# google/nerfactor

Hardware: AMD Instinct MI355X
Metric: rays/sec (NeRF coarse+fine render, 64+128 samples/ray) (higher is better)
Workload: dtype bf16; 1 GPU; lego_3072-shaped NeRF coarse+fine MLP render, 800x800 rays/view, 64+128 samples (BASELINE.json configs[1]); rays_per_view=640000, n_samples_coarse=64, n_samples_fine=128, kernel_variant=7

## Files before the change

nerfactor_amd/_capi.py:

```python
import ctypes
import os

import torch

_HERE = os.path.dirname(os.path.abspath(__file__))
LIB_PATH = os.path.join(_HERE, 'libnfx.so')
if os.environ.get('NFX_LIB_PATH'):
    LIB_PATH = os.environ['NFX_LIB_PATH']

PREC_BF16, PREC_FP32, PREC_FP32_NATIVE = 0, 1, 2
ACT_NONE, ACT_RELU, ACT_SIGMOID, ACT_SOFTPLUS = 0, 1, 2, 3
IN_XYZ, IN_XYZ_LDIR, IN_Z_RUSINK = 0, 1, 2

if not os.path.exists(LIB_PATH):
    raise ImportError(
        "%s not found: build it with `python -m nerfactor_amd.build` (or __graft_entry__.build()); "
        "nerfactor_amd has no fallback path." % LIB_PATH)

lib = ctypes.CDLL(LIB_PATH)

_p = ctypes.c_void_p
_i = ctypes.c_int
_i64 = ctypes.c_int64
_f = ctypes.c_float
# ... 45 lines not shown
    'nfx_nerf_mlp_bwd': (_i, [_p, _p, _p, _i64, _i, _p, _i, _p, _p, _sz, _pp, _pp, _p]),
    'nfx_brdf_train_packed_bytes': (_sz, []),
    'nfx_brdf_pack_train_weights': (_i, [_pp, _pp, _i, _i, _p, _sz]),
    'nfx_brdf_spec_bwd_workspace_bytes': (_sz, [_i, _i64]),
    'nfx_brdf_spec_bwd': (_i, [_p, _p, _p, _p, _i, _p, _i, _p, _i, _i64, _p, _p, _p, _p, _sz, _p]),
    'nfx_brdf_spec_bwd_list_bytes': (_sz, [_i64, _i]),
    'nfx_brdf_spec_bwd_rows': (_i, [_p, _p, _p, _p, _i, _p, _i, _p, _i, _i64, _p, _p, _p, _p, _sz, _p, _sz, _p]),
    'nfx_brdf_rows_fwd': (_i, [_p, _i, _p, _i64, _i, _p, _i, _p, _p]),
    'nfx_brdf_rows_bwd_workspace_bytes': (_sz, [_i, _i64, _i]),
    'nfx_brdf_rows_bwd': (_i, [_p, _i, _p, _i64, _i, _p, _i, _p, _p, _sz, _p, _pp, _pp, _p]),
    'nfx_shade_bwd_workspace_bytes': (_sz, [_i]),
    'nfx_shade_bwd': (_i, [_p, _p, _p, _p, _p, _p, _f, _f, _p, _p, _p, _p, _i64, _i, _i, _p, _p, _p, _p, _p, _p,
                           _p, _p, _sz, _p]),
    'nfx_l2_normalize_rows': (_i, [_p, _p, _i64, _i, _f, _p]),
    'nfx_l2_normalize_rows_bwd': (_i, [_p, _p, _p, _i64, _i, _f, _p]),
    'nfx_light_smoothness': (_i, [_p, _i, _i, _f, _f, _p, _p, _p]),
    'nfx_pair_loss_fwd': (_i, [_p, _i, _p, _f, _i64, _p, _p]),
    'nfx_pair_loss_bwd': (_i, [_p, _i, _p, _f, _i64, _p, _p]),
    'nfx_pack_gather': (_i, [_p, _p, _i64, _p, _p]),
    'nfx_amsgrad_step': (_i, [_p, _p, _p, _p, _p, _i64, _f, _f, _f, _f, _i64, _p]),
    'nfx_amsgrad_step_size': (_f, [_f, _f, _f, _i64]),
    'nfx_amsgrad_step_dev': (_i, [_p, _p, _p, _p, _p, _i64, _p, _f, _f, _f, _p]),
    'nfx_nerf_sigma_fwd': (_i, [_p, _p, _p, _i64, _i, _p, _i, _p, _p]),
    'nfx_lvis_fwd_rows': (_i, [_p, _p, _i64, _f, _p, _i, _p, _i, _p, _sz, _p, _p, _p, _p]),
    'nfx_zero_rows': (_i, [_p, _p, _i64, _i, _p]),
    'nfx_shade_fwd_rows': (_i, [_p, _p, _p, _p, _p, _p, _f, _f, _p, _p, _p, _p, _p, _i64, _i, _i, _i, _p, _p]),
    'nfx_shade_olat_fwd_rows': (_i, [_p, _p, _p, _p, _p, _p, _f, _f, _p, _p, _p, _p, _f, _f, _i64, _i, _i, _p, _p, _p, _p]),
    'nfx_nerf_refine_select': (_i, [_p, _p, _p, _i64, _i, _f, _f, _f, _f, _i, _p, _p, _p]),
    'nfx_nerf_sigma_refine': (_i, [_p, _p, _p, _i64, _i, _p, _p, _p, _p, _p]),
    'nfx_nerf_sigma_refine_last': (_i, [_p, _p, _p, _i64, _i, _p, _p, _p]),
    'nfx_nerf_sigma_fwd_list': (_i, [_p, _p, _p, _i64, _i, _p, _i, _p, _p, _p, _p]),
    'nfx_occgrid_workspace_bytes': (_sz, [_i64, _i]),
    'nfx_occgrid_select': (_i, [_p, _p, _p, _i64, _i, _p, _i, _p, _p, _p, _p, _sz, _p]),
    'nfx_occgrid_bake': (_i, [_p, _i, _i, _f, _i, _p, _p, _p]),
    'nfx_nerf_geom_packed_bytes': (_sz, [_i]),
    'nfx_nerf_pack_geom_weights': (_i, [_pp, _pp, _i, _p, _sz]),
    'nfx_nerf_sigma_grad': (_i, [_p, _p, _p, _i64, _i, _p, _i, _p, _p]),
    'nfx_nerf_sigma_grad_workspace_bytes': (_sz, [_i64, _i]),
    'nfx_nerf_sigma_grad_rows': (_i, [_p, _p, _p, _i64, _i, _p, _i, _p, _p, _sz, _p]),
    'nfx_selftest_mfma_bf16': (_i, [_p, _p, _p, _p]),
    'nfx_selftest_sincos': (_i, [_p, _i64, _i, _p, _p]),
    'nfx_selftest_tr16': (_i, [_p, _p, _p, _i, _p]),
    'nfx_selftest_wgrad_plan': (_i, [_i, _p, _p, _i64, _p, _p, _p, _p]),
    'nfx_selftest_wgrad_partial_bytes': (_sz, [_i, _p, _p, _i64]),
    'nfx_selftest_wgrad_batch': (_i, [_i, _pp, _pp, _p, _p, _pp, _pp, _i64, _i64, _p, _p, _sz, _p]),
    'nfx_mlp_generic_packed_bytes': (_sz, [_i, _i, _p, _p, _i]),
    'nfx_mlp_generic_pack': (_i, [_pp, _pp, _i, _i, _p, _p, _i, _p, _sz]),
    'nfx_mlp_generic_fwd': (_i, [_p, _i64, _i, _i, _i, _p, _p, _p, _p, _i, _p, _i, _i, _p]),
    'nfx_mlp_generic_train_packed_bytes': (_sz, [_i, _i, _p, _p, _i]),
    'nfx_mlp_generic_pack_train': (_i, [_pp, _pp, _i, _i, _p, _p, _i, _p, _sz]),
    'nfx_mlp_generic_bwd_workspace_bytes': (_sz, [_i64, _i, _i, _p, _p, _i]),
    'nfx_mlp_generic_split_hilo': (_i, [_p, _i, _i, _p, _p, _i, _p]),
    'nfx_brdf_rows_geom_fwd': (_i, [_p, _p, _p, _p, _i, _p, _i, _i64, _i, _p, _i, _p, _p]),
    'nfx_brdf_rows_geom_bwd': (_i, [_p, _p, _p, _i, _p, _i, _i64, _i, _p, _i, _p, _p, _p]),
    'nfx_embed_bwd': (_i, [_p, _i64, _i, _i, _p, _i, _i, _p, _p]),
    'nfx_mlp_generic_bwd': (_i, [_p, _i64, _i, _i, _i, _p, _p, _p, _p, _i, _p, _i, _i, _p, _i, _pp, _pp, _p, _sz, _p]),
    'nfx_embed': (_i, [_p, _p, _p, _i64, _i, _i, _i, _i, _p, _i, _i, _p]),
}

for _name, (_res, _args) in SIGNATURES.items():
    _fn = getattr(lib, _name)
    _fn.restype = _res
    _fn.argtypes = _args


class NfxError(RuntimeError):
    """Raised for any non-zero return of the C-ABI; mirrors how the reference surfaces failures as
    Python exceptions (tf.errors.InvalidArgumentError from tf.debugging.*)."""


def last_error():
    buf = ctypes.create_string_buffer(512)
    lib.nfx_last_error(buf, 512)
    return buf.value.decode()


def check(rc, what):
    if rc != 0:
        raise NfxError("%s failed (%d): %s" % (what, rc, last_error()))


OPTION_KEYS = ('nerf_variant', 'nerf_fold', 'nerf_blocks', 'm128_blocks', 'lvis_variant', 'brdf_variant', 'brdf_ct', 'nerf_bwd',
               'nerf_bwd_nw', 'm128_bwd', 'wgrad_lds', 'wgrad_slabs', 'wgrad_rounds', 'wgrad_narrow', 'wgrad_fused', 'lvis_verify', 'lvis_rows', 'brdf_bwd_rows', 'nerf_bwd_rows', 'sigma_grad_rows', 'sigma_variant',
               'sigma_x3_variant')


def set_option(key, value):
    check(lib.nfx_set_option(key.encode(), int(value)), 'nfx_set_option(%s)' % key)


def unset_option(key):
    check(lib.nfx_unset_option(key.encode()), 'nfx_unset_option(%s)' % key)


def get_option(key):
    v, isset = _i(0), _i(0)
    check(lib.nfx_get_option(key.encode(), ctypes.byref(v), ctypes.byref(isset)), 'nfx_get_option(%s)' % key)
    return v.value if isset.value else None


class option:

    def __init__(self, key, value):
        self.key, self.value = key, value

    def __enter__(self):
        self.prev = get_option(self.key)
        if self.value is None:
            unset_option(self.key)
        else:
            set_option(self.key, self.value)
        return self

    def __exit__(self, *exc):
        if self.prev is None:
            unset_option(self.key)
        else:
            set_option(self.key, self.prev)
        return False


for _k in OPTION_KEYS:
    _v = os.environ.get('NFX_' + _k.upper())
    if _v not in (None, ''):
        set_option(_k, int(_v))
```

nerfactor_amd/csrc/capi.cpp:

```cpp
#include <hip/hip_runtime.h>
#include <stdarg.h>
#include <stdio.h>
#include <stdlib.h>
#include <string.h>

#include <atomic>
#include <vector>

#include "capi_common.hpp"
#include "nerf_layout.hpp"
#include "nerf_fold_layout.hpp"
#include "pack.hpp"

static thread_local char g_err[512] = "";

int nfx_fail(int code, const char* fmt, ...) {
    va_list ap;
    va_start(ap, fmt);
    vsnprintf(g_err, sizeof(g_err), fmt, ap);
    va_end(ap);
    return code;
}
int nfx_hip_result(int e, const char* what) {
    if (e == 0) return NFX_OK;
    return nfx_fail(NFX_EHIP, "%s: HIP error %d (%s)", what, e, hipGetErrorString((hipError_t)e));
}

extern "C" {
int nfx_version(void) { return 100; }

int nfx_last_error(char* buf, size_t len) {
    if (!buf || len == 0) return NFX_EINVAL;
    strncpy(buf, g_err, len - 1);
    buf[len - 1] = 0;
    return NFX_OK;
}

namespace {
struct Option {
    const char* key;
    std::atomic<int> value;
    std::atomic<int> is_set;
};
Option g_options[] = {
    {"nerf_variant", {0}, {0}},
    {"nerf_fold", {0}, {0}},
    {"nerf_blocks", {0}, {0}},
    {"m128_blocks", {0}, {0}},
    {"lvis_variant", {0}, {0}},
    {"lvis_verify", {0}, {0}},
    {"lvis_rows", {0}, {0}},
    {"brdf_bwd_rows", {0}, {0}},
    {"sigma_variant", {0}, {0}},
    {"sigma_x3_variant", {0}, {0}},
    {"sigma_grad_rows", {0}, {0}},
    {"nerf_bwd_rows", {0}, {0}},
    {"brdf_variant", {0}, {0}},
    {"brdf_ct", {0}, {0}},
    {"nerf_bwd", {0}, {0}},
    {"nerf_bwd_nw", {0}, {0}},
    {"m128_bwd", {0}, {0}},
    {"wgrad_lds", {0}, {0}},
    {"wgrad_slabs", {0}, {0}},
    {"wgrad_rounds", {0}, {0}},
    {"wgrad_narrow", {0}, {0}},
    {"wgrad_fused", {0}, {0}},
    {"wgrad_splits", {0}, {0}},
    {"wgrad_map", {0}, {0}},
};
Option* find_option(const char* key) {
    if (!key) return nullptr;
    for (Option& o : g_options)
        if (strcmp(o.key, key) == 0) return &o;
    return nullptr;
}
}

int nfx_option_int(const char* key, int dflt) {
    Option* o = find_option(key);
    return o && o->is_set.load(std::memory_order_acquire) ? o->value.load(std::memory_order_relaxed) : dflt;
}
int nfx_set_option(const char* key, int value) {
    Option* o = find_option(key);
    if (!o) return nfx_fail(NFX_EINVAL, "nfx_set_option: unknown option '%s'", key ? key : "(null)");
    o->value.store(value, std::memory_order_relaxed);
    o->is_set.store(1, std::memory_order_release);
    return NFX_OK;
}
int nfx_unset_option(const char* key) {
    Option* o = find_option(key);
    if (!o) return nfx_fail(NFX_EINVAL, "nfx_unset_option: unknown option '%s'", key ? key : "(null)");
    o->is_set.store(0, std::memory_order_release);
    return NFX_OK;
}
int nfx_get_option(const char* key, int* value, int* is_set) {
    Option* o = find_option(key);
    if (!o || !value) return nfx_fail(NFX_EINVAL, "nfx_get_option: unknown option '%s' or null output", key ? key : "(null)");
    *value = o->value.load(std::memory_order_relaxed);
    if (is_set) *is_set = o->is_set.load(std::memory_order_acquire);
    return NFX_OK;
}

size_t nfx_nerf_packed_bytes(int prec) {
    if (prec == NFX_PREC_BF16) return nfx::nerf::kBlobBytes;
    if (prec == NFX_PREC_FP32) return (size_t)nfx::nerf::kBlobBytes + nfx::nerf::kWeightBytes;
    return 0;
}

static int pack_nerf_fragments(const float* const kernels[12], const float* const biases[12], uint8_t* w0, float* b) {
    using namespace nfx;
    using namespace nfx::pack;
    uint8_t* w = w0;
    const Seg pe_xyz{kPosEnc, 10, 0, nullptr};
    const Seg hid256{kHidden, 256, 0, nullptr};
    w += pack_layer_bf16({pe_xyz}, {{kernels[0], biases[0], 256}}, 8, 8, w, b + nerf::kBiasL0);
    for (int l = 1; l <= 7; ++l) {
        float* bl = b + nerf::kBiasL0 + 256 * l;
        if (l == 5) {
            const Seg pe_skip{kPosEnc, 10, 256, nullptr};
            w += pack_layer_bf16({hid256, pe_skip}, {{kernels[5], biases[5], 256}}, 8, 24, w, bl);
        } else {
            w += pack_layer_bf16({hid256}, {{kernels[l], biases[l], 256}}, 8, 16, w, bl);
        }
    }
    w += pack_layer_bf16({hid256}, {{kernels[9], biases[9], 256}, {kernels[8], biases[8], 1}}, 9, 16, w,
                         b + nerf::kBiasBott);
    const Seg pe_view{kPosEnc, 4, 256, nullptr};
    w += pack_layer_bf16({hid256, pe_view}, {{kernels[10], biases[10], 128}}, 4, 24, w, b + nerf::kBiasRgb0);
    const Seg hid128{kHidden, 128, 0, nullptr};
    w += pack_layer_bf16({hid128}, {{kernels[11], biases[11], 3}}, 1, 8, w, b + nerf::kBiasRgb1);
    return w == w0 + nerf::kWeightBytes ? NFX_OK : NFX_EINVAL;
}

int nfx_nerf_pack_weights(const float* const kernels[12], const float* const biases[12], int prec,
                          void* blob, size_t blob_bytes) {
    using namespace nfx;
    REQUIRE(kernels && biases && blob, "nfx_nerf_pack_weights: null argument");
// ... 78 lines not shown
        if (variant == 6)
            return nfx_hip_result(nfx_launch_nerf_mlp_bf16_v6(rayo, rayd, z, n_pts, n_samples, blob, rgbs, blocks,
                                                              0, (hipStream_t)stream),
                                  "nerf_mlp_fwd(bf16, v6)");
        if (variant != 0 && variant != 1)
            return nfx_fail(NFX_EINVAL, "nfx_nerf_mlp_fwd: NFX_NERF_VARIANT %d is not built (0, 1, 6, 7, 8)", variant);
        return nfx_hip_result(nfx_launch_nerf_mlp_bf16(rayo, rayd, z, n_pts, n_samples, blob, rgbs, variant,
                                                       blocks, (hipStream_t)stream),
                              "nerf_mlp_fwd(bf16)");
    }
    if (prec == NFX_PREC_FP32)
        return nfx_hip_result(nfx_launch_nerf_mlp_x3(rayo, rayd, z, n_pts, n_samples, blob, rgbs, blocks, (hipStream_t)stream),
                              "nerf_mlp_fwd(fp32 via 3 x bf16)");
    return nfx_fail(NFX_EINVAL, "nfx_nerf_mlp_fwd: bad prec %d", prec);
}

size_t nfx_nerf_fold_workspace_bytes(void) { return nfx::nerf::fold::kBlobBytes; }

int nfx_nerf_fold_blob(const void* blob, void* workspace, size_t workspace_bytes, void* stream) {
    REQUIRE(blob && workspace, "nfx_nerf_fold_blob: null pointer");
    REQUIRE(workspace_bytes >= nfx_nerf_fold_workspace_bytes(), "nfx_nerf_fold_blob: workspace too small (%zu < %zu)",
            workspace_bytes, nfx_nerf_fold_workspace_bytes());
    if (!ALIGNED(blob, 16) || !ALIGNED(workspace, 16))
        return nfx_fail(NFX_EALIGN, "nfx_nerf_fold_blob: blob and workspace must be 16-byte aligned");
    const uintptr_t b = (uintptr_t)blob, w = (uintptr_t)workspace;
    REQUIRE(b + nfx::nerf::kBlobBytes <= w || w + nfx_nerf_fold_workspace_bytes() <= b,
            "nfx_nerf_fold_blob: the workspace overlaps the blob");
    return nfx_hip_result(nfx_launch_nerf_fold(blob, workspace, (hipStream_t)stream), "nerf_fold_blob");
}

int nfx_nerf_mlp_fwd_folded(const float* rayo, const float* rayd, const float* z, int64_t n_rays, int n_samples,
                            const void* blob, void* workspace, size_t workspace_bytes, float* rgbs, void* stream) {
    REQUIRE(n_rays >= 0 && n_samples >= 1, "nfx_nerf_mlp_fwd_folded: bad shape (%lld rays, %d samples)",
            (long long)n_rays, n_samples);
    if (n_rays == 0) return NFX_OK;
    REQUIRE(rayo && rayd && z && blob && rgbs, "nfx_nerf_mlp_fwd_folded: null pointer");
    if (!ALIGNED(rgbs, 16)) return nfx_fail(NFX_EALIGN, "nfx_nerf_mlp_fwd_folded: rgbs must be 16-byte aligned");
    const int rc = nfx_nerf_fold_blob(blob, workspace, workspace_bytes, stream);
    if (rc) return rc;
    const long long n_pts = (long long)n_rays * n_samples;
    const int blocks = nfx_option_int("nerf_blocks", 256);
    const int variant = nfx_option_int("nerf_variant", 7);
    if (variant == 6 || variant == 7 || variant == 8)
        return nfx_hip_result(nfx_launch_nerf_mlp_bf16_v6_fold(rayo, rayd, z, n_pts, n_samples, workspace, rgbs, blocks,
                                                               variant == 8 ? 2 : variant == 7 ? 1 : 0, (hipStream_t)stream),
                              "nerf_mlp_fwd_folded(bf16, v6-8)");
    if (variant != 0 && variant != 1)
        return nfx_fail(NFX_EINVAL, "nfx_nerf_mlp_fwd_folded: NFX_NERF_VARIANT %d is not built (0, 1, 6, 7, 8)", variant);
    return nfx_hip_result(nfx_launch_nerf_mlp_bf16_fold(rayo, rayd, z, n_pts, n_samples, workspace, rgbs, variant, blocks,
                                                        (hipStream_t)stream),
                          "nerf_mlp_fwd_folded(bf16)");
}

int nfx_composite_fwd(const float* rgbs, const float* z, const float* rayd, const float* noise,
                      int64_t n_rays, int n_samples, int white_bg, float* rgb, float* occu, float* depth,
                      float* disp, float* weights, void* stream) {
    REQUIRE(n_rays >= 0 && n_samples >= 1, "nfx_composite_fwd: bad shape");
    if (n_rays == 0) return NFX_OK;
    REQUIRE(rgbs && z && rayd, "nfx_composite_fwd: null input");
    if (!ALIGNED(rgbs, 16)) return nfx_fail(NFX_EALIGN, "nfx_composite_fwd: rgbs must be 16-byte aligned");
    return nfx_hip_result(nfx_launch_composite(rgbs, z, rayd, noise, n_rays, n_samples, white_bg, rgb, occu,
                                               depth, disp, weights, (hipStream_t)stream),
                          "composite_fwd");
}

int nfx_nerf_surface_fwd(const float* sigma, const float* z, const float* rayo, const float* rayd, int64_t n_rays,
                         int n_samples, float occu_thres, int quantize_alpha, float* alpha, float* xyz, float* depth,
                         float* occu, void* stream) {
    REQUIRE(n_rays >= 0 && n_samples >= 1, "nfx_nerf_surface_fwd: bad shape (%lld rays, %d samples)", (long long)n_rays,
            n_samples);
    REQUIRE(occu_thres == occu_thres, "nfx_nerf_surface_fwd: occu_thres is NaN");
    if (n_rays == 0) return NFX_OK;
    REQUIRE(sigma && z && rayo && rayd, "nfx_nerf_surface_fwd: null input");
    REQUIRE(alpha && xyz && depth, "nfx_nerf_surface_fwd: null output (only occu may be NULL)");
    return nfx_hip_result(nfx_launch_surface(sigma, z, rayo, rayd, n_rays, n_samples, occu_thres, quantize_alpha ? 1 : 0, alpha,
                                             xyz, depth, occu, (hipStream_t)stream),
                          "nerf_surface_fwd");
}

int nfx_sample_fine(const float* z, const float* weights, int64_t n_rays, int n_coarse, int n_fine,
                    const float* u, float* z_all, void* stream) {
    REQUIRE(n_rays >= 0, "nfx_sample_fine: n_rays < 0");
    REQUIRE(n_coarse <= 258, "nfx_sample_fine: at most 258 coarse samples (256 pdf bins), got %d", n_coarse);
    REQUIRE(n_coarse >= 3 && n_fine >= 2, "nfx_sample_fine: need n_coarse >= 3 and n_fine >= 2 (got %d, %d)",
            n_coarse, n_fine);
    REQUIRE((size_t)4 * (2 * (n_coarse - 1) + n_coarse + n_fine) * 4 <= 64 * 1024,
            "nfx_sample_fine: n_coarse + n_fine too large for one workgroup's LDS");
    if (n_rays == 0) return NFX_OK;
    REQUIRE(z && weights && z_all, "nfx_sample_fine: null pointer");
    return nfx_hip_result(
            nfx_launch_sample_fine(z, weights, n_rays, n_coarse, n_fine, u, z_all, (hipStream_t)stream),
            "sample_fine");
}

int nfx_selftest_mfma_bf16(const float* a, const float* b, float* d, void* stream) {
    REQUIRE(a && b && d, "nfx_selftest_mfma_bf16: null pointer");
    return nfx_hip_result(nfx_launch_selftest_mfma(a, b, d, (hipStream_t)stream), "selftest_mfma");
}
int nfx_selftest_tr16(const float* h, const float* z, float* d, int mode, void* stream) {
    REQUIRE(d && (mode == 1 || (h && z)), "nfx_selftest_tr16: null pointer");
    return nfx_hip_result(nfx_launch_selftest_tr16(h, z, d, mode, (hipStream_t)stream), "selftest_tr16");
}
int nfx_selftest_sincos(const float* in, int64_t n, int which, float* out, void* stream) {
    REQUIRE(n >= 0 && (n == 0 || (in && out)), "nfx_selftest_sincos: bad arguments");
    return nfx_hip_result(nfx_launch_selftest_sincos(in, n, which, out, (hipStream_t)stream), "selftest_sincos");
}

}
```

nerfactor_amd/csrc/launchers.hpp:

```cpp
#pragma once
#include <hip/hip_runtime.h>
#include <stddef.h>
#include <stdint.h>

#include "../../include/nfx.h"

namespace nfx::generic { struct Args; struct EmbedArgs; struct BwdArgs; struct WgradArgs; }
namespace nfx::rowsgeom { struct Args; }
namespace nfx::geo { struct Points; }

struct nfx_wgrad_call {
    const void* xt;
    const void* zt;
    int k_in, n_out;
    float* dw;
    float* db;
};

extern "C" {
int nfx_option_int(const char* key, int dflt);
int nfx_brdf_train_blob_bytes(void);
int nfx_launch_brdf_spec_bwd(const float* xyz, const float* cam, const float* normal, const float* z, int z_dim, const float* lxyz,
                             int n_lights, const void* blob, long long n, const float* dspec, float* d_z, float* d_normal, void* workspace,
                             int max_blocks, hipStream_t st, void* list_ws);
// ... 8 lines not shown
int nfx_launch_merl_sphere(const float* xyz, const float* normal, long long n, const float* cam3, const void* table4, const float* lxyz,
                           const float* lweight, int n_lights, float* rgb, int* idx, hipStream_t st);
int nfx_launch_pair_loss(int bwd, const nfx_loss_term* terms, int n_terms, const float* alpha, float bg, long long n, float* loss,
                         const float* dloss, hipStream_t st);
int nfx_launch_lvis_v2(const float* xyz, long long n, const float* lxyz, int n_lights, const float* pre, const void* blob_main, float* lvis,
                       int ct, int max_blocks, hipStream_t st, const int* out_row, int* nan_flag);
int nfx_launch_brdf_spec_v2(const float* xyz, const float* cam, const float* normal, const float* z, int z_dim, const float* lxyz,
                            int n_lights, const void* blob, long long n, float* spec, int ct, int max_blocks, hipStream_t st);
int nfx_launch_brdf_spec_v3(const float* xyz, const float* cam, const float* normal, const float* z, int z_dim, const float* lxyz,
                            int n_lights, const void* blob, long long n, float* spec, int ct, int geo, int max_blocks, hipStream_t st);
int nfx_launch_mlp128_xyz(const float* xyz, long long n, float xyz_scale, const void* blob, int out_dim, int out_act, float post_scale,
                          float post_bias, float* out, int max_blocks, hipStream_t st);
int nfx_launch_lvis_pre(const float* xyz, long long n, float xyz_scale, const void* blob_pre, float* pre, int max_blocks, hipStream_t st);
int nfx_launch_lvis(const float* xyz, long long n, const float* lxyz, int n_lights, const float* pre, const void* blob_main, float* lvis,
                    int max_blocks, hipStream_t st);
int nfx_launch_brdf_spec(const float* xyz, const float* cam, const float* normal, const float* z, int z_dim, const float* lxyz,
                         int n_lights, const void* blob, long long n, float* spec, int max_blocks, hipStream_t st);
int nfx_launch_mlp128_bwd(int in_kind, const float* xyz, const float* xyz_dir, long long n, float xyz_scale, const float* lxyz,
                          int n_lights, const void* blob, int out_dim, int out_act, float post_scale, const float* dout, void* wsp,
                          long long ld, int max_blocks, hipStream_t st);
int nfx_mlp128_train_feats(int in_kind);
int nfx_mlp128_train_blob_bytes(int in_kind);
size_t nfx_mlp128_fused_partial_floats(int in_kind, int grid);
int nfx_mlp128_fused_grid(int in_kind, long long n, int n_lights, int max_blocks);
int nfx_launch_mlp128_bwd_fused(int in_kind, const float* xyz, const float* xyz_dir, long long n, float xyz_scale, const float* lxyz,
                                int n_lights, int n_heads, const void* const* blobs, const int* out_dims, const int* out_acts,
                                const float* post_scales, const float* const* douts, float* partial, int grid, float* const* dk,
                                float* const* db, hipStream_t st);
int nfx_mlp128_x3_weight_bytes(int in_kind);
int nfx_launch_mlp128_x3(int in_kind, const float* xyz, const float* xyz_dir, const float* lxyz, const float* cam, const float* normal,
                         const float* z, int z_dim, long long n, int n_lights, float xyz_scale, const void* blob, int out_dim, int out_act,
                         float post_scale, float post_bias, float* out, int max_blocks, hipStream_t st);
int nfx_generic_fwd_m0(const nfx::generic::Args* args, int nw, int grid, int lds, hipStream_t st);
int nfx_generic_fwd_m1(const nfx::generic::Args* args, int nw, int grid, int lds, hipStream_t st);
int nfx_generic_fwd_m2(const nfx::generic::Args* args, int nw, int grid, int lds, hipStream_t st);
int nfx_generic_bwd_m0(const nfx::generic::BwdArgs* ba, const nfx::generic::WgradArgs* wa, int nw, int grid, int lds, hipStream_t st);
int nfx_generic_bwd_m1(const nfx::generic::BwdArgs* ba, const nfx::generic::WgradArgs* wa, int nw, int grid, int lds, hipStream_t st);
int nfx_generic_bwd_m2(const nfx::generic::BwdArgs* ba, const nfx::generic::WgradArgs* wa, int nw, int grid, int lds, hipStream_t st);
int nfx_launch_mlp_generic(const nfx::generic::Args* args, int max_blocks, hipStream_t st);
int nfx_launch_mlp_generic_bwd(const nfx::generic::BwdArgs* ba, const nfx::generic::WgradArgs* wa, int max_blocks, hipStream_t st);
int nfx_launch_split_hilo(void* frags, long long n_frags, hipStream_t st);
int nfx_launch_embed_bwd(const nfx::generic::EmbedArgs* a, const float* d_out, float* dv, hipStream_t st);
int nfx_launch_embed(const nfx::generic::EmbedArgs* a, hipStream_t st);
size_t nfx_nerf_bwd_list_bytes(long long n_pts);
int nfx_launch_nerf_bwd(const float* rayo, const float* rayd, const float* z, long long n_pts, int n_samples, const void* blob,
                        const float* d_rgbs, void* wsp, long long ld, int max_blocks, hipStream_t st, void* list_ws);
int nfx_launch_nerf_fold(const void* blob, void* out, hipStream_t stream);
int nfx_launch_nerf_sigma_grad(const nfx::geo::Points* pts, const void* blob, float* out, int max_blocks, hipStream_t st);
int nfx_launch_select_density(const float* sigma, long long n_pts, float* out, void* list_ws, hipStream_t st);
int nfx_launch_nerf_sigma_geo(const float* rayo, const float* rayd, const float* z, long long n_pts, int n_samples, const void* blob,
                              float* out, int max_blocks, hipStream_t st);
int nfx_launch_nerf_sigma_grad_x3(const nfx::geo::Points* pts, const void* blob, float* out, int max_blocks, hipStream_t st);
int nfx_launch_nerf_sigma_x3(const nfx::geo::Points* pts, const void* blob, float* out, int max_blocks, hipStream_t st);
int nfx_launch_nerf_mlp_bf16(const float* rayo, const float* rayd, const float* z, long long n_pts, int n_samples, const void* blob,
                             float* out, int variant, int max_blocks, hipStream_t stream);
int nfx_launch_nerf_mlp_bf16_fold(const float* rayo, const float* rayd, const float* z, long long n_pts, int n_samples, const void* blob,
                                  float* out, int variant, int max_blocks, hipStream_t stream);
int nfx_launch_nerf_mlp_bf16_v6(const float* rayo, const float* rayd, const float* z, long long n_pts, int n_samples, const void* blob,
                                float* out, int max_blocks, int dma_mode, hipStream_t stream);
int nfx_launch_nerf_mlp_bf16_v6_fold(const float* rayo, const float* rayd, const float* z, long long n_pts, int n_samples, const void* blob,
                                     float* out, int max_blocks, int dma_mode, hipStream_t stream);
int nfx_launch_nerf_mlp_x3(const float* rayo, const float* rayd, const float* z, long long n_pts, int n_samples, const void* blob,
                           float* out, int max_blocks, hipStream_t stream);
int nfx_launch_nerf_sigma_v6(const float* rayo, const float* rayd, const float* z, long long n_pts, int n_samples, const void* blob,
                             float* out, int max_blocks, hipStream_t stream);
int nfx_launch_nerf_sigma_v6_list(const float* rayo, const float* rayd, const float* z, long long capacity, int n_samples, const void* blob,
                                  float* out, const int* list, const int* count, int max_blocks, hipStream_t stream);
int nfx_launch_nerf_sigma_x3_pipe(const nfx::geo::Points* pts, const void* blob, float* out, int max_blocks, hipStream_t st);
size_t nfx_occgrid_list_bytes(long long n_pts);
int nfx_launch_occgrid_select(const float* rayo, const float* rayd, const float* z, long long n_rays, int n_samples, const uint32_t* bits,
                              int res, const float* box, const float* bbox, float* out, void* ws, hipStream_t st);
int nfx_launch_occgrid_bake(const float* sigma, int res, int probes, float margin, int dilate, uint32_t* bits, uint32_t* ws,
                            hipStream_t st);
int nfx_launch_pack_gather(const float* src, const int* map, long long n_words, void* blob, hipStream_t st);
int nfx_launch_l2_normalize3(const float* in, float* out, long long n, float eps, hipStream_t st);
int nfx_launch_gen_z(float near, float far, int n_samples, long long n_rays, int lin_in_disp, const float* u, float* z, hipStream_t st);
int nfx_launch_composite(const float* rgbs, const float* z, const float* rayd, const float* noise, long long n_rays, int S, int white_bg,
                         float* rgb, float* occu, float* depth, float* disp, float* w, hipStream_t st);
int nfx_launch_surface(const float* sigma, const float* z, const float* rayo, const float* rayd, long long n_rays, int S, float occu_thres,
                       int quantize, float* alpha, float* xyz, float* depth, float* occu, hipStream_t st);
int nfx_launch_refine_select(const float* rgbs, const float* z, const float* rayd, long long n_rays, int S, float t_min, float a_lo,
                             float a_hi, float sigma_margin, int dilate, int* list, int* count, hipStream_t st);
int nfx_launch_sample_fine(const float* z, const float* w, long long n_rays, int nc, int nf, const float* u, float* z_all, hipStream_t st);
int nfx_launch_composite_bwd(const float* rgbs, const float* z, const float* rayd, const float* noise, long long n_rays, int n_samples,
                             int white_bg, const float* d_rgb, float* d_rgbs, hipStream_t st);
int nfx_launch_scatter_rows(const float* src, const int* row_of, long long n_all, int d, float* dst, hipStream_t st);
int nfx_launch_zero_rows(float* dst, const int* row_of, long long n_all, int d, hipStream_t st);
int nfx_launch_nonfinite(const float* x, long long n, int* flag, hipStream_t st);
int nfx_launch_l2_normalize_rows(int bwd, const float* x, const float* dy, float* out, long long n, int d, float eps, hipStream_t st);
int nfx_launch_light_smoothness(const float* light, int H, int W, float tv_w, float achro_w, float* loss, float* grad, hipStream_t st);
int nfx_launch_selftest_tr16(const float* h, const float* z, float* d, int mode, hipStream_t st);
int nfx_launch_selftest_mfma(const float* a, const float* b, float* d, hipStream_t st);
int nfx_launch_selftest_sincos(const float* in, long long n, int which, float* out, hipStream_t st);
size_t nfx_shade_olat_lds_bytes(int n_lights);
int nfx_launch_shade(const float* xyz, const float* cam, const float* normal, const float* albedo, const float* rough, const float* spec,
                     float spec_scale, float f0, const float* lvis, const float* lxyz, const float* lareas, const float* lights,
                     long long n, int n_lights, int n_probes, int to_srgb, float* out, hipStream_t st, const int* lvis_row);
int nfx_launch_shade_olat(const float* xyz, const float* cam, const float* normal, const float* albedo, const float* rough,
                          const float* spec, float spec_scale, float f0, const float* lvis, const float* lxyz, const float* lareas,
                          float olat_inten, float ambient, long long n, int n_lights, int to_srgb, float* out, hipStream_t st,
                          const int* lvis_row, const int* out_row, int* nan_flag);
int nfx_launch_dir2rusink(const float* a, const float* b, long long n, float* out, hipStream_t st);
size_t nfx_shade_bwd_lds_bytes(int n_lights, int with_light_grad);
int nfx_launch_shade_bwd(const float* xyz, const float* cam, const float* normal, const float* albedo, const float* rough,
                         const float* spec, float spec_scale, float f0, const float* lvis, const float* lxyz, const float* lareas,
                         const float* light, long long n, int n_lights, int to_srgb, const float* drgb, float* d_albedo, float* d_rough,
                         float* d_spec, float* d_normal, float* d_lvis, float* d_light, void* workspace, hipStream_t st);
int nfx_launch_amsgrad(float* p, const float* g, float* m, float* v, float* vhat, long long n, float lr_t, float b1, float b2, float eps,
                       hipStream_t st);
int nfx_launch_amsgrad_dev(float* p, const float* g, float* m, float* v, float* vhat, long long n, const float* lr_t_dev, float b1,
                           float b2, float eps, hipStream_t st);
size_t nfx_wgrad_partial_bytes(const nfx_wgrad_call* calls, int n_calls, long long rows);
int nfx_launch_wgrad_batch_counted(const nfx_wgrad_call* calls, int n_calls, long long ld, long long rows, void* partial, const int* count,
                                   hipStream_t st);
int nfx_launch_wgrad_batch(const nfx_wgrad_call* calls, int n_calls, long long ld, long long rows, void* partial, hipStream_t st);
void nfx_wgrad_plan_of(const nfx_wgrad_call* calls, int n_calls, long long rows, int* form, long long* slab, int* n_slabs);
int nfx_wgrad_max_calls(void);
int nfx_wgrad_counted_ok(long long rows);
}
```

nerfactor_amd/csrc/raymarch.hip:

```cpp
#include "nfx_common.hpp"
#include "launchers.hpp"

namespace nfx {

__global__ void l2_normalize3_kernel(const float* __restrict__ in, float* __restrict__ out,
                                     long long n, float eps) {
    const long long i = (long long)blockIdx.x * blockDim.x + threadIdx.x;
    if (i >= n) return;
    const float x = in[3 * i], y = in[3 * i + 1], z = in[3 * i + 2];
    const float sq = x * x + y * y + z * z;
    const float inv = 1.0f / sqrtf(fmaxf(sq, eps));
    out[3 * i] = x * inv;
    out[3 * i + 1] = y * inv;
    out[3 * i + 2] = z * inv;
}

__device__ __forceinline__ float linspace01(int i, int n) { return (float)i * (1.0f / (float)(n - 1)); }

__device__ __forceinline__ float z_of_t(float t, float near, float far, int lin_in_disp) {
    if (lin_in_disp) return 1.0f / (1.0f / near * (1.0f - t) + 1.0f / far * t);
    return near * (1.0f - t) + far * t;
}

__global__ void gen_z_kernel(float near, float far, int n_samples, long long n_rays,
// ... 324 lines not shown
#pragma unroll
    for (int k = 0; k < kMaxSeg; ++k) wv[k] = (64 * k + lane < nb) ? wr[1 + 64 * k + lane] : 0.f;
    float denom = 0.f;
#pragma unroll
    for (int k = 0; k < kMaxSeg; ++k) {
        const int cnt = nb - 64 * k < 64 ? nb - 64 * k : 64;
        for (int i = 0; i < cnt; ++i) denom += __shfl(wv[k], i, 64);
    }
    denom += 1e-5f;
    float pdf[kMaxSeg], cv[kMaxSeg];
#pragma unroll
    for (int k = 0; k < kMaxSeg; ++k) {
        pdf[k] = wv[k] / denom;
        cv[k] = 0.f;
    }
    float acc = 0.f;
#pragma unroll
    for (int k = 0; k < kMaxSeg; ++k) {
        const int cnt = nb - 64 * k < 64 ? nb - 64 * k : 64;
        for (int i = 0; i < cnt; ++i) {
            acc += __shfl(pdf[k], i, 64);
            if (lane == i) cv[k] = acc;
        }
    }
    if (lane == 0) cdf[0] = 0.f;
#pragma unroll
    for (int k = 0; k < kMaxSeg; ++k)
        if (64 * k + lane < nb) cdf[1 + 64 * k + lane] = cv[k];
    __syncthreads();
    for (int i = lane; i < nf; i += 64) {
        const float uu = u ? u[rc * nf + i] : linspace01(i, nf);
        int lo = 0, hi = ncdf;
        while (lo < hi) {
            const int m = (lo + hi) >> 1;
            if (cdf[m] <= uu) lo = m + 1; else hi = m;
        }
        const int ind = lo;
        const int below = ind - 1 > 0 ? ind - 1 : 0;
        const int above = ind < ncdf - 1 ? ind : ncdf - 1;
        const float cb = cdf[below], ca = cdf[above];
        float den = ca - cb;
        den = den < 1e-5f ? 1.0f : den;
        const float t = (uu - cb) / den;
        const float vb = mid[below], va = mid[above];
        zall[nc + i] = vb + t * (va - vb);
    }
    __syncthreads();
    if (u == nullptr) {
        const float* zc = zall;
        const float* zf = zall + nc;
        for (int i = lane; i < ntot; i += 64) {
            const float v = zall[i];
            int lo = 0, hi, rank;
            if (i < nc) {
                hi = nf;
                while (lo < hi) {
                    const int m = (lo + hi) >> 1;
                    if (zf[m] < v) lo = m + 1; else hi = m;
                }
                rank = i + lo;
            } else {
                hi = nc;
                while (lo < hi) {
                    const int m = (lo + hi) >> 1;
                    if (zc[m] <= v) lo = m + 1; else hi = m;
                }
                rank = (i - nc) + lo;
            }
            if (active) z_all[ray * ntot + rank] = v;
        }
        return;
    }
    for (int i = lane; i < ntot; i += 64) {
        const float v = zall[i];
        int rank = 0;
        for (int j = 0; j < ntot; ++j) {
            const float o = zall[j];
            rank += (o < v) || (o == v && j < i);
        }
        if (active) z_all[ray * ntot + rank] = v;
    }
}

}

extern "C" {
int nfx_launch_l2_normalize3(const float* in, float* out, long long n, float eps, hipStream_t st) {
    if (n <= 0) return 0;
    hipLaunchKernelGGL(nfx::l2_normalize3_kernel, dim3((unsigned)((n + 255) / 256)), dim3(256), 0, st,
                       in, out, n, eps);
    return (int)hipGetLastError();
}
int nfx_launch_gen_z(float near, float far, int n_samples, long long n_rays, int lin_in_disp,
                     const float* u, float* z, hipStream_t st) {
    const long long tot = n_rays * n_samples;
    if (tot <= 0) return 0;
    hipLaunchKernelGGL(nfx::gen_z_kernel, dim3((unsigned)((tot + 255) / 256)), dim3(256), 0, st, near,
                       far, n_samples, n_rays, lin_in_disp, u, z);
    return (int)hipGetLastError();
}
int nfx_launch_composite(const float* rgbs, const float* z, const float* rayd, const float* noise,
                         long long n_rays, int S, int white_bg, float* rgb, float* occu, float* depth,
                         float* disp, float* w, hipStream_t st) {
    if (n_rays <= 0) return 0;
    hipLaunchKernelGGL(nfx::composite_kernel, dim3((unsigned)((n_rays + 3) / 4)), dim3(256), 0, st,
                       (const float4*)rgbs, z, rayd, noise, n_rays, S, white_bg ? 1.0f : 0.0f, rgb,
                       occu, depth, disp, w);
    return (int)hipGetLastError();
}
int nfx_launch_surface(const float* sigma, const float* z, const float* rayo, const float* rayd, long long n_rays, int S,
                       float occu_thres, int quantize, float* alpha, float* xyz, float* depth, float* occu, hipStream_t st) {
    if (n_rays <= 0) return 0;
    hipLaunchKernelGGL(nfx::surface_kernel, dim3((unsigned)((n_rays + 3) / 4)), dim3(256), 0, st, sigma, z, rayo, rayd,
                       n_rays, S, occu_thres, quantize, alpha, xyz, depth, occu);
    return (int)hipGetLastError();
}
int nfx_launch_refine_select(const float* rgbs, const float* z, const float* rayd, long long n_rays, int S, float t_min,
                             float a_lo, float a_hi, float sigma_margin, int dilate, int* list, int* count, hipStream_t st) {
    hipError_t e = hipMemsetAsync(count, 0, sizeof(int), st);
    if (e != hipSuccess) return (int)e;
    if (n_rays <= 0) return 0;
    hipLaunchKernelGGL(nfx::refine_select_kernel, dim3((unsigned)((n_rays + 4 * nfx::kSelRays - 1) / (4 * nfx::kSelRays))), dim3(256), 0, st,
                       (const float4*)rgbs, z, rayd, n_rays, S, t_min, a_lo, a_hi, sigma_margin, dilate, list, count);
    return (int)hipGetLastError();
}
int nfx_launch_sample_fine(const float* z, const float* w, long long n_rays, int nc, int nf,
                           const float* u, float* z_all, hipStream_t st) {
    if (n_rays <= 0) return 0;
    const size_t lds = (size_t)4 * (2 * (nc - 1) + nc + nf) * sizeof(float);
    hipLaunchKernelGGL(nfx::sample_fine_kernel, dim3((unsigned)((n_rays + 3) / 4)), dim3(256), lds, st,
                       z, w, n_rays, nc, nf, u, z_all);
    return (int)hipGetLastError();
}
int nfx_launch_composite_bwd(const float* rgbs, const float* z, const float* rayd, const float* noise,
                             long long n_rays, int n_samples, int white_bg, const float* d_rgb, float* d_rgbs,
                             hipStream_t st) {
    if (n_rays <= 0) return 0;
    const size_t lds = (size_t)4 * 2 * n_samples * sizeof(float);
    if (lds > 64 * 1024) {
        hipError_t e = hipFuncSetAttribute(reinterpret_cast<const void*>(nfx::composite_bwd_kernel),
                                           hipFuncAttributeMaxDynamicSharedMemorySize, (int)lds);
        if (e != hipSuccess) return (int)e;
    }
    hipLaunchKernelGGL(nfx::composite_bwd_kernel, dim3((unsigned)((n_rays + 3) / 4)), dim3(256), lds, st,
                       (const float4*)rgbs, z, rayd, noise, n_rays, n_samples, white_bg ? 1.0f : 0.0f, d_rgb,
                       (float4*)d_rgbs);
    return (int)hipGetLastError();
}
}

namespace nfx {
__global__ __launch_bounds__(256) void nonfinite_kernel(const unsigned* __restrict__ x, long long n, int* __restrict__ flag) {
    const long long n4 = n / 4;
    const uint4* x4 = reinterpret_cast<const uint4*>(x);
    bool bad = false;
    for (long long i = (long long)blockIdx.x * 256 + threadIdx.x; i < n4; i += (long long)gridDim.x * 256) {
        const uint4 v = x4[i];
        bad = bad || (v.x & 0x7f800000u) == 0x7f800000u || (v.y & 0x7f800000u) == 0x7f800000u ||
              (v.z & 0x7f800000u) == 0x7f800000u || (v.w & 0x7f800000u) == 0x7f800000u;
    }
    if (blockIdx.x == 0 && threadIdx.x < (int)(n - 4 * n4))
        bad = bad || (x[4 * n4 + threadIdx.x] & 0x7f800000u) == 0x7f800000u;
    if (__ballot(bad) != 0 && (threadIdx.x & 63) == 0) atomicOr(flag, 1);
}

__global__ __launch_bounds__(256) void zero_rows_kernel(float4* __restrict__ dst, const int* __restrict__ row_of, unsigned n_elems,
                                                        unsigned per_row) {
    for (unsigned i = blockIdx.x * 256u + threadIdx.x; i < n_elems; i += gridDim.x * 256u)
        if (row_of[i / per_row] < 0) dst[i] = make_float4(0.f, 0.f, 0.f, 0.f);
}

template <typename T>
__global__ __launch_bounds__(256) void scatter_rows_kernel(const T* __restrict__ src, const int* __restrict__ row_of,
                                                           unsigned n_elems, unsigned per_row, T* __restrict__ dst) {
    T zero;
    __builtin_memset(&zero, 0, sizeof(T));
    for (unsigned i = blockIdx.x * 256u + threadIdx.x; i < n_elems; i += gridDim.x * 256u) {
        const unsigned row = i / per_row, col = i - row * per_row;
        const int r = row_of[row];
        dst[i] = r >= 0 ? src[(unsigned long long)r * per_row + col] : zero;
    }
}
}

extern "C" int nfx_launch_scatter_rows(const float* src, const int* row_of, long long n_all, int d, float* dst,
                                       hipStream_t st) {
    if (n_all <= 0 || d <= 0) return 0;
    const bool v4 = d % 4 == 0 && (reinterpret_cast<uintptr_t>(src) % 16 == 0) && (reinterpret_cast<uintptr_t>(dst) % 16 == 0);
    const long long per_row = v4 ? d / 4 : d, n_elems = n_all * per_row;
    if (n_elems > (1ll << 31) + (1ll << 20)) return (int)hipErrorInvalidValue;
    long long blocks = (n_elems + 255) / 256;
    if (blocks > 8192) blocks = 8192;
    if (v4)
        hipLaunchKernelGGL(nfx::scatter_rows_kernel<float4>, dim3((unsigned)blocks), dim3(256), 0, st,
                           reinterpret_cast<const float4*>(src), row_of, (unsigned)n_elems, (unsigned)per_row,
                           reinterpret_cast<float4*>(dst));
    else
        hipLaunchKernelGGL(nfx::scatter_rows_kernel<float>, dim3((unsigned)blocks), dim3(256), 0, st, src, row_of,
                           (unsigned)n_elems, (unsigned)per_row, dst);
    return (int)hipGetLastError();
}

extern "C" int nfx_launch_zero_rows(float* dst, const int* row_of, long long n_all, int d, hipStream_t st) {
    if (n_all <= 0 || d <= 0) return 0;
    const long long per_row = d / 4;
    const long long rows_per_call = ((1ll << 31) - 1) / per_row;
    for (long long r0 = 0; r0 < n_all; r0 += rows_per_call) {
        const long long rows = n_all - r0 < rows_per_call ? n_all - r0 : rows_per_call;
        const long long n_elems = rows * per_row;
        long long blocks = (n_elems + 255) / 256;
        if (blocks > 8192) blocks = 8192;
// ... 16 lines not shown
```

Before: 5.152 million rays/s.

## Add 64-ray-per-block sample_fine kernel with binary-search merge ranking

Adds a new hierarchical-sampling kernel that handles 64 rays per 256-thread block and is used by default. It stages weights in LDS rows, does per-ray normalisation and CDF prefix sums one thread per ray, and inverts the CDF with binary search. For deterministic u it ranks the merged coarse+fine z values by binary search over the two sorted halves instead of the O(n^2) all-pairs count. It targets the old 4-rays-per-block layout and the quadratic sort, at the cost of more LDS per block and serial per-thread prefix sums.

```diff
diff --git a/nerfactor_amd/_capi.py b/nerfactor_amd/_capi.py
--- a/nerfactor_amd/_capi.py
+++ b/nerfactor_amd/_capi.py
@@ -151,7 +151,7 @@
 
 OPTION_KEYS = ('nerf_variant', 'nerf_fold', 'nerf_blocks', 'm128_blocks', 'lvis_variant', 'brdf_variant', 'brdf_ct', 'nerf_bwd',
                'nerf_bwd_nw', 'm128_bwd', 'wgrad_lds', 'wgrad_slabs', 'wgrad_rounds', 'wgrad_narrow', 'wgrad_fused', 'lvis_verify', 'lvis_rows', 'brdf_bwd_rows', 'nerf_bwd_rows', 'sigma_grad_rows', 'sigma_variant',
-               'sigma_x3_variant')
+               'sigma_x3_variant', 'sample_fine_variant')
 
 
 def set_option(key, value):
diff --git a/nerfactor_amd/csrc/capi.cpp b/nerfactor_amd/csrc/capi.cpp
--- a/nerfactor_amd/csrc/capi.cpp
+++ b/nerfactor_amd/csrc/capi.cpp
@@ -53,6 +53,7 @@
     {"brdf_bwd_rows", {0}, {0}},
     {"sigma_variant", {0}, {0}},
     {"sigma_x3_variant", {0}, {0}},
+    {"sample_fine_variant", {0}, {0}},
     {"sigma_grad_rows", {0}, {0}},
     {"nerf_bwd_rows", {0}, {0}},
     {"brdf_variant", {0}, {0}},
@@ -297,10 +298,14 @@
                     const float* u, float* z_all, void* stream) {
     REQUIRE(n_rays >= 0, "nfx_sample_fine: n_rays < 0");
     REQUIRE(n_coarse <= 258, "nfx_sample_fine: at most 258 coarse samples (256 pdf bins), got %d", n_coarse);
-    REQUIRE(n_coarse >= 3 && n_fine >= 2, "nfx_sample_fine: need n_coarse >= 3 and n_fine >= 2 (got %d, %d)",
+    REQUIRE(n_coarse >= 3 && n_fine >= (u ? 1 : 2), "nfx_sample_fine: need n_coarse >= 3 and n_fine >= 2, or >= 1 with u (got %d, %d)",
             n_coarse, n_fine);
     REQUIRE((size_t)4 * (2 * (n_coarse - 1) + n_coarse + n_fine) * 4 <= 64 * 1024,
             "nfx_sample_fine: n_coarse + n_fine too large for one workgroup's LDS");
+    if (nfx_option_int("sample_fine_variant", 1) != 0)
+        REQUIRE(nfx_sample_fine_rows_lds(n_coarse, n_fine) <= 160 * 1024,
+                "nfx_sample_fine: %d coarse + %d fine samples need %zu bytes of LDS for a block of rays, the CU has %d", n_coarse,
+                n_fine, nfx_sample_fine_rows_lds(n_coarse, n_fine), 160 * 1024);
     if (n_rays == 0) return NFX_OK;
     REQUIRE(z && weights && z_all, "nfx_sample_fine: null pointer");
     return nfx_hip_result(
diff --git a/nerfactor_amd/csrc/launchers.hpp b/nerfactor_amd/csrc/launchers.hpp
--- a/nerfactor_amd/csrc/launchers.hpp
+++ b/nerfactor_amd/csrc/launchers.hpp
@@ -114,6 +114,7 @@
 int nfx_launch_refine_select(const float* rgbs, const float* z, const float* rayd, long long n_rays, int S, float t_min, float a_lo,
                              float a_hi, float sigma_margin, int dilate, int* list, int* count, hipStream_t st);
 int nfx_launch_sample_fine(const float* z, const float* w, long long n_rays, int nc, int nf, const float* u, float* z_all, hipStream_t st);
+size_t nfx_sample_fine_rows_lds(int nc, int nf);
 int nfx_launch_composite_bwd(const float* rgbs, const float* z, const float* rayd, const float* noise, long long n_rays, int n_samples,
                              int white_bg, const float* d_rgb, float* d_rgbs, hipStream_t st);
 int nfx_launch_scatter_rows(const float* src, const int* row_of, long long n_all, int d, float* dst, hipStream_t st);
diff --git a/nerfactor_amd/csrc/raymarch.hip b/nerfactor_amd/csrc/raymarch.hip
--- a/nerfactor_amd/csrc/raymarch.hip
+++ b/nerfactor_amd/csrc/raymarch.hip
@@ -430,6 +430,146 @@
     }
 }
 
+constexpr int kFineRows = 64;
+constexpr size_t kFineLdsMax = 160 * 1024;
+__host__ __device__ constexpr int fine_row_stride(int nc) { return (nc - 1) | 1; }
+__host__ __device__ constexpr size_t fine_rows_lds_floats(int nc, int nf) {
+    return (size_t)kFineRows * fine_row_stride(nc) + 4 * (size_t)(nc + nf);
+}
+
+__device__ __forceinline__ void wave_lds_sync() {
+    __builtin_amdgcn_fence(__ATOMIC_RELEASE, "wavefront");
+    __builtin_amdgcn_wave_barrier();
+    __builtin_amdgcn_fence(__ATOMIC_ACQUIRE, "wavefront");
+}
+
+__global__ __launch_bounds__(256) void sample_fine_rows_kernel(
+    const float* __restrict__ z, const float* __restrict__ weights, long long n_rays, int nc, int nf,
+    const float* __restrict__ u, float* __restrict__ z_all) {
+    extern __shared__ __attribute__((aligned(16))) char smem_raw[];
+    float* rows = reinterpret_cast<float*>(smem_raw);
+    const int lane = threadIdx.x & 63, wave = threadIdx.x >> 6;
+    const int nb = nc - 2;
+    const int ncdf = nc - 1;
+    const int ntot = nc + nf;
+    const int stride = fine_row_stride(nc);
+    float* zall = rows + (size_t)kFineRows * stride + (size_t)wave * ntot;
+    const long long ray0 = (long long)blockIdx.x * kFineRows;
+    const int n_here = n_rays - ray0 < kFineRows ? (int)(n_rays - ray0) : kFineRows;
+
+    for (int r = wave; r < n_here; r += 4) {
+        const float* wr = weights + (ray0 + r) * nc;
+        float* row = rows + r * stride;
+        for (int i = 1 + lane; i <= nb; i += 64) row[i] = wr[i];
+    }
+    __syncthreads();
+    if ((int)threadIdx.x < n_here) {
+        float* row = rows + threadIdx.x * stride;
+        float denom = 0.f;
+#pragma unroll 8
+        for (int i = 1; i <= nb; ++i) denom += row[i];
+        denom += 1e-5f;
+        row[0] = denom;
+    }
+    __syncthreads();
+    for (int r = wave; r < n_here; r += 4) {
+        float* row = rows + r * stride;
+        const float denom = row[0];
+        for (int i = 1 + lane; i <= nb; i += 64) row[i] = row[i] / denom;
+    }
+    __syncthreads();
+    if ((int)threadIdx.x < n_here) {
+        float* row = rows + threadIdx.x * stride;
+        float acc = 0.f;
+        row[0] = 0.f;
+#pragma unroll 8
+        for (int i = 1; i <= nb; ++i) {
+            acc += row[i];
+            row[i] = acc;
+        }
+    }
+    __syncthreads();
+    for (int r = wave; r < n_here; r += 4) {
+        const long long ray = ray0 + r;
+        const float* cdf = rows + r * stride;
+        const float* zr = z + ray * nc;
+        for (int i = lane; i < nc; i += 64) zall[i] = zr[i];
+        wave_lds_sync();
+        for (int i = lane; i < nf; i += 64) {
+            const float uu = u ? u[ray * nf + i] : linspace01(i, nf);
+            int lo = 0, hi = ncdf;
+            while (lo < hi) {
+                const int m = (lo + hi) >> 1;
+                if (cdf[m] <= uu) lo = m + 1; else hi = m;
+            }
+            const int ind = lo;
+            const int below = ind - 1 > 0 ? ind - 1 : 0;
+            const int above = ind < ncdf - 1 ? ind : ncdf - 1;
+            const float cb = cdf[below], ca = cdf[above];
+            float den = ca - cb;
+            den = den < 1e-5f ? 1.0f : den;
+            const float t = (uu - cb) / den;
+            const float vb = 0.5f * (zall[below + 1] + zall[below]);
+            const float va = 0.5f * (zall[above + 1] + zall[above]);
+            zall[nc + i] = vb + t * (va - vb);
+        }
+        wave_lds_sync();
+        if (u == nullptr) {
+            const float* zc = zall;
+            const float* zf = zall + nc;
+            for (int i = lane; i < ntot; i += 64) {
+                const float v = zall[i];
+                int lo = 0, hi, rank;
+                if (i < nc) {
+                    hi = nf;
+                    while (lo < hi) {
+                        const int m = (lo + hi) >> 1;
+                        if (zf[m] < v) lo = m + 1; else hi = m;
+                    }
+                    rank = i + lo;
+                } else {
+                    hi = nc;
+                    while (lo < hi) {
+                        const int m = (lo + hi) >> 1;
+                        if (zc[m] <= v) lo = m + 1; else hi = m;
+                    }
+                    rank = (i - nc) + lo;
+                }
+                z_all[ray * ntot + rank] = v;
+            }
+        } else {
+            for (int i = lane; i < ntot; i += 64) {
+                const float v = zall[i];
+                int rank = 0;
+                for (int j = 0; j < ntot; ++j) {
+                    const float o = zall[j];
+                    rank += (o < v) || (o == v && j < i);
+                }
+                z_all[ray * ntot + rank] = v;
+            }
+        }
+        wave_lds_sync();
+    }
+}
+
+static int launch_sample_fine_rows(const float* z, const float* w, long long n_rays, int nc, int nf, const float* u,
+                                   float* z_all, hipStream_t st) {
+    const size_t lds = fine_rows_lds_floats(nc, nf) * sizeof(float);
+    if (lds > kFineLdsMax) return (int)hipErrorInvalidValue;
+    if (lds > 64 * 1024) {
+        hipError_t e = hipFuncSetAttribute(reinterpret_cast<const void*>(sample_fine_rows_kernel),
+                                           hipFuncAttributeMaxDynamicSharedMemorySize, (int)lds);
+        if (e != hipSuccess) return (int)e;
+    }
+    hipLaunchKernelGGL(sample_fine_rows_kernel, dim3((unsigned)((n_rays + kFineRows - 1) / kFineRows)), dim3(256), lds, st,
+                       z, w, n_rays, nc, nf, u, z_all);
+    return (int)hipGetLastError();
+}
+
+}
+
+extern "C" size_t nfx_sample_fine_rows_lds(int nc, int nf) {
+    return nfx::fine_rows_lds_floats(nc, nf) * sizeof(float);
 }
 
 extern "C" {
@@ -475,6 +615,7 @@
 int nfx_launch_sample_fine(const float* z, const float* w, long long n_rays, int nc, int nf,
                            const float* u, float* z_all, hipStream_t st) {
     if (n_rays <= 0) return 0;
+    if (nfx_option_int("sample_fine_variant", 1) != 0) return nfx::launch_sample_fine_rows(z, w, n_rays, nc, nf, u, z_all, st);
     const size_t lds = (size_t)4 * (2 * (nc - 1) + nc + nf) * sizeof(float);
     hipLaunchKernelGGL(nfx::sample_fine_kernel, dim3((unsigned)((n_rays + 3) / 4)), dim3(256), lds, st,
                        z, w, n_rays, nc, nf, u, z_all);
```

Measured after the change: 5.177 million rays/s (median of 6 runs). Within noise of the previous version (+0.5%).

## Add grouped sample_fine kernel with per-lane CDF and binary-search merge

Applied to the files above, without the earlier changes.

Adds a new sample_fine variant in which each wave handles eight rays. Weights and z are staged into LDS with a padded pitch, and each lane builds the CDF for one ray. The inverse-CDF lookup and the merge of coarse and fine samples now use batched binary searches instead of O(n^2) rank counting. It is enabled by default once the ray count passes a threshold and the LDS footprint fits. The aim is to cut per-ray serial work and the quadratic sort cost, at the price of more LDS use and lower occupancy.

```diff
diff --git a/nerfactor_amd/_capi.py b/nerfactor_amd/_capi.py
--- a/nerfactor_amd/_capi.py
+++ b/nerfactor_amd/_capi.py
@@ -151,7 +151,7 @@
 
 OPTION_KEYS = ('nerf_variant', 'nerf_fold', 'nerf_blocks', 'm128_blocks', 'lvis_variant', 'brdf_variant', 'brdf_ct', 'nerf_bwd',
                'nerf_bwd_nw', 'm128_bwd', 'wgrad_lds', 'wgrad_slabs', 'wgrad_rounds', 'wgrad_narrow', 'wgrad_fused', 'lvis_verify', 'lvis_rows', 'brdf_bwd_rows', 'nerf_bwd_rows', 'sigma_grad_rows', 'sigma_variant',
-               'sigma_x3_variant')
+               'sigma_x3_variant', 'sample_fine_variant')
 
 
 def set_option(key, value):
diff --git a/nerfactor_amd/csrc/capi.cpp b/nerfactor_amd/csrc/capi.cpp
--- a/nerfactor_amd/csrc/capi.cpp
+++ b/nerfactor_amd/csrc/capi.cpp
@@ -53,6 +53,7 @@
     {"brdf_bwd_rows", {0}, {0}},
     {"sigma_variant", {0}, {0}},
     {"sigma_x3_variant", {0}, {0}},
+    {"sample_fine_variant", {0}, {0}},
     {"sigma_grad_rows", {0}, {0}},
     {"nerf_bwd_rows", {0}, {0}},
     {"brdf_variant", {0}, {0}},
diff --git a/nerfactor_amd/csrc/raymarch.hip b/nerfactor_amd/csrc/raymarch.hip
--- a/nerfactor_amd/csrc/raymarch.hip
+++ b/nerfactor_amd/csrc/raymarch.hip
@@ -430,6 +430,188 @@
     }
 }
 
+__device__ __forceinline__ void wave_lds_fence() {
+    asm volatile("" ::: "memory");
+    __builtin_amdgcn_wave_barrier();
+}
+
+template <int K, bool STRICT>
+__device__ __forceinline__ void bsearch_k(const float* list, int len, const float (&v)[K], int (&lo)[K]) {
+    int hi[K];
+#pragma unroll
+    for (int k = 0; k < K; ++k) {
+        lo[k] = 0;
+        hi[k] = len;
+    }
+    const int sure = 31 - __clz(len + 1);
+    for (int it = 0; it < sure; ++it) {
+        int m[K];
+        float x[K];
+#pragma unroll
+        for (int k = 0; k < K; ++k) {
+            m[k] = (lo[k] + hi[k]) >> 1;
+            x[k] = list[m[k]];
+        }
+#pragma unroll
+        for (int k = 0; k < K; ++k) {
+            const bool right = STRICT ? x[k] < v[k] : x[k] <= v[k];
+            lo[k] = right ? m[k] + 1 : lo[k];
+            hi[k] = right ? hi[k] : m[k];
+        }
+    }
+    if (32 - __clz(len) > sure) {
+#pragma unroll
+        for (int k = 0; k < K; ++k) {
+            const float x = list[lo[k]];
+            const bool right = (STRICT ? x < v[k] : x <= v[k]) && lo[k] < hi[k];
+            lo[k] = right ? lo[k] + 1 : lo[k];
+        }
+    }
+}
+
+template <int K, bool RANDOM_U>
+__device__ __forceinline__ void inverse_cdf_k(const float* cdf, const float* zc, int ncdf, const float* u_ray, int nf, int i0,
+                                              float* zf) {
+    int ind[K];
+    float uu[K];
+#pragma unroll
+    for (int k = 0; k < K; ++k) {
+        const int i = i0 + 64 * k;
+        uu[k] = RANDOM_U ? (i < nf ? u_ray[i] : 0.f) : linspace01(i, nf);
+    }
+    bsearch_k<K, false>(cdf, ncdf, uu, ind);
+#pragma unroll
+    for (int k = 0; k < K; ++k) {
+        if (i0 + 64 * k >= nf) continue;
+        const int below = ind[k] - 1 > 0 ? ind[k] - 1 : 0;
+        const int above = ind[k] < ncdf - 1 ? ind[k] : ncdf - 1;
+        const float cb = cdf[below], ca = cdf[above];
+        float den = ca - cb;
+        den = den < 1e-5f ? 1.0f : den;
+        const float t = (uu[k] - cb) / den;
+        const float vb = 0.5f * (zc[below + 1] + zc[below]), va = 0.5f * (zc[above + 1] + zc[above]);
+        zf[i0 + 64 * k] = vb + t * (va - vb);
+    }
+}
+
+template <int K, bool STRICT>
+__device__ __forceinline__ void merge_rank_k(const float* own, int n_own, const float* other, int n_other, int i0,
+                                             float* __restrict__ out) {
+    int cnt[K];
+    float v[K];
+#pragma unroll
+    for (int k = 0; k < K; ++k) {
+        const int i = i0 + 64 * k;
+        v[k] = own[i < n_own ? i : 0];
+    }
+    bsearch_k<K, STRICT>(other, n_other, v, cnt);
+#pragma unroll
+    for (int k = 0; k < K; ++k)
+        if (i0 + 64 * k < n_own) out[i0 + 64 * k + cnt[k]] = v[k];
+}
+
+constexpr int kSampleFineGroup = 8;
+constexpr long long kSampleFineGroupMinRays = 16384;
+constexpr size_t kSampleFineGroupMaxLds = 64 * 1024;
+
+template <int G, bool RANDOM_U>
+__global__ __launch_bounds__(256) void sample_fine_group_kernel(
+    const float* __restrict__ z, const float* __restrict__ weights, long long n_rays, int nc, int nf,
+    const float* __restrict__ u, float* __restrict__ z_all) {
+    static_assert(G >= 1 && G <= 64, "one lane per ray of the group");
+    extern __shared__ __attribute__((aligned(16))) char smem_raw[];
+    const int lane = threadIdx.x & 63, wave = threadIdx.x >> 6;
+    const int nb = nc - 2, ncdf = nc - 1, ntot = nc + nf;
+    const int pitch = nc | 1;
+    float* zcs = reinterpret_cast<float*>(smem_raw) + (size_t)wave * (G * nc + nf + G * pitch);
+    float* zf = zcs + G * nc;
+    float* tile = zf + nf;
+    const long long ray0 = ((long long)blockIdx.x * 4 + wave) * G;
+    if (ray0 >= n_rays) return;
+    const int rows = n_rays - ray0 < G ? (int)(n_rays - ray0) : G;
+
+    const float* wg = weights + ray0 * nc;
+    const float* zg = z + ray0 * nc;
+    for (int i0 = 0; i0 < nc; i0 += 64) {
+        const int i = i0 + lane, ic = i < nc ? i : nc - 1;
+        for (int r0 = 0; r0 < rows; r0 += 4) {
+            float wv[4], zv[4];
+#pragma unroll
+            for (int k = 0; k < 4; ++k) {
+                const int at = (r0 + k < rows ? r0 + k : rows - 1) * nc + ic;
+                wv[k] = wg[at];
+                zv[k] = zg[at];
+            }
+#pragma unroll
+            for (int k = 0; k < 4; ++k)
+                if (i < nc && r0 + k < rows) {
+                    tile[(r0 + k) * pitch + i] = wv[k];
+                    zcs[(r0 + k) * nc + i] = zv[k];
+                }
+        }
+    }
+    wave_lds_fence();
+    float* row = tile + (lane < rows ? lane : 0) * pitch;
+    float denom = 0.f;
+    if (lane < rows) {
+        for (int i = 0; i < nb; ++i) denom += row[1 + i];
+        denom += 1e-5f;
+    }
+    for (int r = 0; r < rows; ++r) {
+        const float d = __int_as_float(__builtin_amdgcn_readlane(__float_as_int(denom), r));
+        for (int i0 = 0; i0 < nb; i0 += 64)
+            if (i0 + lane < nb) tile[r * pitch + 1 + i0 + lane] = tile[r * pitch + 1 + i0 + lane] / d;
+    }
+    wave_lds_fence();
+    if (lane < rows) {
+        float acc = 0.f;
+        for (int i = 0; i < nb; ++i) {
+            acc += row[1 + i];
+            row[1 + i] = acc;
+        }
+        row[0] = 0.f;
+    }
+    wave_lds_fence();
+
+    for (int r = 0; r < rows; ++r) {
+        const long long ray = ray0 + r;
+        const float* zc = zcs + r * nc;
+        const float* cdf = tile + r * pitch;
+        const float* u_ray = RANDOM_U ? u + ray * nf : nullptr;
+        for (int i0 = 0; i0 < nf; i0 += 128) {
+            if (i0 + 64 < nf) inverse_cdf_k<2, RANDOM_U>(cdf, zc, ncdf, u_ray, nf, i0 + lane, zf);
+            else inverse_cdf_k<1, RANDOM_U>(cdf, zc, ncdf, u_ray, nf, i0 + lane, zf);
+        }
+        wave_lds_fence();
+        float* out = z_all + ray * ntot;
+        if (!RANDOM_U) {
+            for (int i0 = 0; i0 < nc; i0 += 128) {
+                if (i0 + 64 < nc) merge_rank_k<2, true>(zc, nc, zf, nf, i0 + lane, out);
+                else merge_rank_k<1, true>(zc, nc, zf, nf, i0 + lane, out);
+            }
+            for (int i0 = 0; i0 < nf; i0 += 128) {
+                if (i0 + 64 < nf) merge_rank_k<2, false>(zf, nf, zc, nc, i0 + lane, out);
+                else merge_rank_k<1, false>(zf, nf, zc, nc, i0 + lane, out);
+            }
+        } else {
+            for (int i = lane; i < ntot; i += 64) {
+                const float v = i < nc ? zc[i] : zf[i - nc];
+                int rank = 0;
+                for (int j = 0; j < nc; ++j) {
+                    const float o = zc[j];
+                    rank += (o < v) || (o == v && j < i);
+                }
+                for (int j = 0; j < nf; ++j) {
+                    const float o = zf[j];
+                    rank += (o < v) || (o == v && nc + j < i);
+                }
+                out[rank] = v;
+            }
+        }
+        wave_lds_fence();
+    }
+}
+
 }
 
 extern "C" {
@@ -475,6 +657,15 @@
 int nfx_launch_sample_fine(const float* z, const float* w, long long n_rays, int nc, int nf,
                            const float* u, float* z_all, hipStream_t st) {
     if (n_rays <= 0) return 0;
+    const int variant = nfx_option_int("sample_fine_variant", -1);
+    constexpr int g = nfx::kSampleFineGroup;
+    const size_t lds_group = (size_t)4 * ((size_t)(nc + (nc | 1)) * g + nf) * sizeof(float);
+    if (lds_group <= nfx::kSampleFineGroupMaxLds && (variant == 1 || (variant < 0 && n_rays >= nfx::kSampleFineGroupMinRays))) {
+        auto kernel = u ? nfx::sample_fine_group_kernel<g, true> : nfx::sample_fine_group_kernel<g, false>;
+        hipLaunchKernelGGL(kernel, dim3((unsigned)((n_rays + 4 * g - 1) / (4 * g))), dim3(256), lds_group, st, z, w, n_rays, nc,
+                           nf, u, z_all);
+        return (int)hipGetLastError();
+    }
     const size_t lds = (size_t)4 * (2 * (nc - 1) + nc + nf) * sizeof(float);
     hipLaunchKernelGGL(nfx::sample_fine_kernel, dim3((unsigned)((n_rays + 3) / 4)), dim3(256), lds, st,
                        z, w, n_rays, nc, nf, u, z_all);
```

Result: no change. 5.275 million rays/s before, 5.298 million rays/s after (median of 6 runs) (+0.4%).
